# iamgroot42/A-LINK

Hardware: AMD Instinct MI355X
Metric: 112x112 face embeddings/sec (IR-ResNet-100 ArcFace, 512-d, L2-normalised) (higher is better)
Workload: dtype bf16

## Files before the change

a-link_amd/csrc/front_c64.hip:

```cpp
#include "conv_device.h"

namespace alink {
namespace {

typedef __attribute__((__vector_size__(4 * sizeof(int)))) int i32x4;

__device__ __forceinline__ void lds_done_then_barrier() {
    asm volatile("s_waitcnt lgkmcnt(0)\n\ts_barrier" ::: "memory");
}

template <int A>
struct IC { static constexpr int a = A; };

constexpr int NT = 256;
constexpr int W = 112, H = 112;
constexpr int P = 2;
constexpr int RING = 8;
constexpr int BR = 4;
constexpr int BPI = H / BR;
constexpr int PITCH = (W + 2) * 128;
constexpr int XBYTES = RING * PITCH;
constexpr int TBYTES = 11 * 64 * 4;
constexpr int IMPX = 32;
constexpr int IMROWB = W * IMPX;
constexpr int IMROWS = 8;
constexpr int TPWV = 7;
constexpr size_t lds_bytes() { return (size_t)XBYTES + TBYTES + IMROWS * IMROWB + 16; }

template <typename T, int LAYOUT, bool AMAX, bool STAMP>
__global__ __launch_bounds__(NT, 1) void front_c64_kernel(const ConvParams p, const StemParams s, T* __restrict__ xs) {
    typedef typename Vec8<T>::type vec8;
    auto prelu = [](float v, float slope) __attribute__((always_inline)) {
        const float w = v * slope;
        return AMAX ? __builtin_fmaxf(v, w) : (v > 0.f ? v : w);
    };
    extern __shared__ __attribute__((aligned(16))) char smem[];
    char* const imring = smem + XBYTES + TBYTES;

    const int tid = threadIdx.x, lane = tid & 63;
    const int wave = __builtin_amdgcn_readfirstlane(tid >> 6);
    const int ph = wave >> 1, ch = wave & 1;
    const int q = lane >> 4, lr = lane & 15;

    for (int i = tid; i < RING * 16; i += NT) {
        const int slot = i >> 4, side = (i >> 3) & 1, piece = i & 7;
        *(uint4*)(smem + slot * PITCH + (side ? (W + 1) * 128 : 0) + piece * 16) = uint4{0u, 0u, 0u, 0u};
    }
    for (int i = tid; i < IMROWS * IMROWB / 16; i += NT)
        *(uint4*)(imring + i * 16) = uint4{0u, 0u, 0u, 0u};
    float* const ebias = (float*)(smem + XBYTES);
    float* const ealpha = ebias + 9 * 64;
    for (int i = tid; i < 9 * 64; i += NT) ebias[i] = p.bias[i];
    float* const salpha = ealpha + 64;
    for (int i = tid; i < 64; i += NT) { ealpha[i] = p.alpha[i]; salpha[i] = s.alpha[i]; }

    const T* __restrict__ gw = (const T*)p.wgt;
    vec8 wr[2][9][2];
#pragma unroll
    for (int ct = 0; ct < 2; ++ct)
#pragma unroll
        for (int tap = 0; tap < 9; ++tap)
#pragma unroll
            for (int ks = 0; ks < 2; ++ks)
                wr[ct][tap][ks] = *(const vec8*)(gw + (size_t)(ch * 32 + 16 * ct + lr) * 576 + tap * 64 + ks * 32 + 8 * q);
    const int d = delta(lr);
    int loff[3][2];
#pragma unroll
    for (int kx = 0; kx < 3; ++kx)
#pragma unroll
        for (int ks = 0; ks < 2; ++ks)
            loff[kx][ks] = (d + kx) * 128 + ((((ks << 2) | q) ^ (((d + kx) >> 1) & 7)) << 4);

    vec8 swf[2][2];
#pragma unroll
    for (int t = 0; t < 2; ++t)
#pragma unroll
        for (int st = 0; st < 2; ++st) swf[t][st] = *(const vec8*)((const T*)s.wgt + (16 * (2 * ch + t) + lr) * 64 + st * 32 + 8 * q);
    float sbi[8];
#pragma unroll
    for (int i = 0; i < 8; ++i) sbi[i] = s.bias[16 * q + 8 * ch + i];
    const int rec_off = lr * IMPX + (q & 1) * 16;
    const int sw_off = (lr + 1) * 128 + (((2 * q + ch) ^ (((lr + 1) >> 1) & 7)) << 4);

    int goff[3], soff[3], prow[3];
    float ssub[3];
    {
        float sb0 = s.sub[0], sb1 = s.sub[1], sb2 = s.sub[2];
        asm volatile("" : "+s"(sb0), "+s"(sb1), "+s"(sb2));
#pragma unroll
        for (int jj = 0; jj < 3; ++jj) {
            const int i = tid + NT * jj;
            const bool valid = i < 672;
            const int r = i >= 336 ? 1 : 0, e = valid ? i - 336 * r : 0;
            int c, ix;
            if (LAYOUT == ALINK_LAYOUT_NCHW_F32) { c = e / W; ix = e - c * W; }
            else                                 { ix = e / 3; c = e - ix * 3; }
            const int cn = s.flip ? 2 - c : c;
            ssub[jj] = cn == 0 ? sb0 : (cn == 1 ? sb1 : sb2);
            goff[jj] = LAYOUT == ALINK_LAYOUT_NCHW_F32 ? c * H * W + ix : e;
            soff[jj] = valid ? (ix + 1) * IMPX + cn * 2 : -1;
            prow[jj] = r;
        }
    }
    constexpr int ROWP = LAYOUT == ALINK_LAYOUT_NCHW_F32 ? W : W * 3;
    char* const sink = imring + IMROWS * IMROWB;
    auto load_pair = [&](int n, int iy0, float (&raw)[3]) __attribute__((always_inline)) {
        const size_t base = (size_t)n * 3 * H * W;
#pragma unroll
        for (int jj = 0; jj < 3; ++jj) {
            int iy = iy0 + prow[jj];
            iy = iy < 0 ? 0 : (iy > H - 1 ? H - 1 : iy);
            const long long idx = (long long)base + iy * ROWP + goff[jj];
            if (LAYOUT == ALINK_LAYOUT_NHWC_U8) raw[jj] = (float)((const uint8_t*)s.in)[idx];
            else                                raw[jj] = ((const float*)s.in)[idx];
        }
    };
    auto store_pair = [&](int iy0, const float (&raw)[3]) __attribute__((always_inline)) {
        char* const rb0 = imring + ((iy0 + 8) & 7) * IMROWB;
        char* const rb1 = imring + ((iy0 + 9) & 7) * IMROWB;
#pragma unroll
        for (int jj = 0; jj < 3; ++jj) {
            const bool ok = (unsigned)(iy0 + prow[jj]) < (unsigned)H;
            const T v = (T)(ok ? (raw[jj] - ssub[jj]) * s.mul : 0.f);
            char* const dst = (prow[jj] ? rb1 : rb0) + soff[jj];
            *(T*)(soff[jj] >= 0 && soff[jj] < W * IMPX ? dst : sink) = v;
            *(T*)(soff[jj] >= 0 ? dst - IMPX + 6 : sink) = v;
            *(T*)(soff[jj] >= 2 * IMPX ? dst - 2 * IMPX + 12 : sink) = v;
        }
    };
    auto stem_rows = [&](int R0, int slot0, int n, int own_lo, int own_hi) __attribute__((always_inline)) {
        const int R = R0 + ph;
        int slot = slot0 + ph;
        if (slot >= RING) slot -= RING;
        const bool inimg = (unsigned)R < (unsigned)H;
        const char* const rbm = imring + ((R + 7) & 7) * IMROWB;
        const char* const rbz = imring + ((R + 8) & 7) * IMROWB;
        const char* const rbp = imring + ((R + 9) & 7) * IMROWB;
        const char* const wa = (q < 2 ? rbm : rbz) + rec_off;
        const char* const wb = rbp + rec_off;
        char* const ob = smem + slot * PITCH + sw_off;
        const bool to_xs = inimg && !(R & 1) && R >= own_lo && R < own_hi && !(lr & 1);
        T* const xrow = xs + ((size_t)(n * (H / 2) + (R >> 1)) * (W / 2) + (lr >> 1)) * 64 + 16 * q + 8 * ch;
        const int keep = inimg ? -1 : 0;
        const f32x4 sal0 = *(const f32x4*)(salpha + 16 * q + 8 * ch), sal1 = *(const f32x4*)(salpha + 16 * q + 8 * ch + 4);
        auto group = [&](auto X0, auto NX) __attribute__((always_inline)) {
            constexpr int x0 = decltype(X0)::a, nx = decltype(NX)::a;
            vec8 pa[nx], pb[nx];
#pragma unroll
            for (int i = 0; i < nx; ++i) {
                pa[i] = *(const vec8*)(wa + 16 * IMPX * (x0 + i));
                pb[i] = *(const vec8*)(wb + 16 * IMPX * (x0 + i));
            }
            f32x4 a0[nx], a1[nx];
#pragma unroll
            for (int i = 0; i < nx; ++i) {
                a0[i] = mfma16<T>(swf[0][0], pa[i], f32x4{sbi[0], sbi[1], sbi[2], sbi[3]});
                a1[i] = mfma16<T>(swf[1][0], pa[i], f32x4{sbi[4], sbi[5], sbi[6], sbi[7]});
            }
#pragma unroll
            for (int i = 0; i < nx; ++i) {
                a0[i] = mfma16<T>(swf[0][1], pb[i], a0[i]);
                a1[i] = mfma16<T>(swf[1][1], pb[i], a1[i]);
            }
#pragma unroll
            for (int i = 0; i < nx; ++i) {
                vec8 o8;
#pragma unroll
                for (int j = 0; j < 4; ++j) {
                    float v0 = a0[i][j], v1 = a1[i][j];
                    v0 = prelu(v0, sal0[j]);
                    v1 = prelu(v1, sal1[j]);
                    o8[j] = (T)v0;
                    o8[4 + j] = (T)v1;
                }
                i32x4 ob4 = __builtin_bit_cast(i32x4, o8);
#pragma unroll
                for (int j = 0; j < 4; ++j) ob4[j] &= keep;
                *(i32x4*)(ob + 2048 * (x0 + i)) = ob4;
                if (to_xs) *(i32x4*)(xrow + (size_t)(8 * (x0 + i)) * 64) = ob4;
            }
        };
        group(IC<0>{}, IC<4>{});
        group(IC<4>{}, IC<3>{});
    };

    auto compute = [&](f32x4 (&acc)[2][TPWV], int s0) __attribute__((always_inline)) {
#pragma unroll
        for (int ct = 0; ct < 2; ++ct)
#pragma unroll
            for (int u = 0; u < TPWV; ++u) acc[ct][u] = f32x4{0.f, 0.f, 0.f, 0.f};
        int sb[3];
#pragma unroll
        for (int ky = 0; ky < 3; ++ky) {
            int slot = s0 + ph + ky;
            if (slot >= RING) slot -= RING;
            sb[ky] = slot * PITCH;
        }
        vec8 pf[2][TPWV];
#pragma unroll
        for (int u = 0; u < TPWV; ++u) pf[0][u] = *(const vec8*)(smem + (sb[0] + loff[0][0]) + 2048 * u);
#pragma unroll
        for (int st = 0; st < 18; ++st) {
            if (st + 1 < 18) {
                const int tn = (st + 1) >> 1, ksn = (st + 1) & 1;
#pragma unroll
                for (int u = 0; u < TPWV; ++u)
                    pf[(st + 1) & 1][u] = *(const vec8*)(smem + (sb[tn / 3] + loff[tn % 3][ksn]) + 2048 * u);
            }
            const int tap = st >> 1, ks = st & 1;
#pragma unroll
            for (int ct = 0; ct < 2; ++ct)
#pragma unroll
                for (int u = 0; u < TPWV; ++u) acc[ct][u] = mfma16<T>(wr[ct][tap][ks], pf[st & 1][u], acc[ct][u]);
        }
    };
    auto epilogue = [&](const f32x4 (&acc)[2][TPWV], int y, long long img_row0) __attribute__((always_inline)) {
        const int rc = y == 0 ? 0 : (y == H - 1 ? 2 : 1);
        const size_t rowoff = (size_t)((img_row0 + y) * W) * 64 + ch * 32 + 8 * q;
        const f32x4 al0 = *(const f32x4*)(ealpha + ch * 32 + 8 * q), al1 = *(const f32x4*)(ealpha + ch * 32 + 8 * q + 4);
#pragma unroll
        for (int u = 0; u < TPWV; ++u) {
            const int x = 16 * u + d;
            const int cls = rc * 3 + (x == 0 ? 0 : (x == W - 1 ? 2 : 1));
            const f32x4 b0 = *(const f32x4*)(ebias + cls * 64 + ch * 32 + 8 * q);
            const f32x4 b1 = *(const f32x4*)(ebias + cls * 64 + ch * 32 + 8 * q + 4);
            float v[8];
#pragma unroll
            for (int j = 0; j < 4; ++j) { v[j] = acc[0][u][j] + b0[j]; v[4 + j] = acc[1][u][j] + b1[j]; }
#pragma unroll
            for (int i = 0; i < 8; ++i) v[i] = prelu(v[i], i < 4 ? al0[i & 3] : al1[i & 3]);
            vec8 o8;
#pragma unroll
            for (int i = 0; i < 8; ++i) o8[i] = (T)v[i];
            *(vec8*)((T*)p.out + rowoff + (size_t)x * 64) = o8;
        }
    };

    unsigned long long t_bar = 0, t_stem = 0, t_main = 0, t_pro = 0, t_a = 0, t_b = 0, t_c = 0, n_pass = 0;
    const unsigned long long t_start = STAMP ? __builtin_amdgcn_s_memtime() : 0;
    const long long nbands = (long long)p.N * BPI;
    const long long b0 = nbands * blockIdx.x / gridDim.x, b1 = nbands * (blockIdx.x + 1) / gridDim.x;
    for (long long band = b0; band < b1;) {
        const int n = (int)(band / BPI), j0 = (int)(band - (long long)n * BPI);
        int rb = BPI - j0;
        if (rb > b1 - band) rb = (int)(b1 - band);
        band += rb;
        const int y0 = j0 * BR, npass = rb * (BR / P), yend = y0 + rb * BR;
        const long long img_row0 = (long long)n * H;

        float raw[3];
        if (STAMP) t_a = __builtin_amdgcn_s_memtime();
        {
            float rawA[3], rawB[3], rawC[3];
            load_pair(n, y0 - 2, rawA);
            load_pair(n, y0, rawB);
            load_pair(n, y0 + 2, rawC);
            load_pair(n, y0 + 4, raw);
            lds_done_then_barrier();
            store_pair(y0 - 2, rawA);
            store_pair(y0, rawB);
            lds_done_then_barrier();
            store_pair(y0 + 2, rawC);
            stem_rows(y0 - 1, 0, n, y0, yend);
            lds_done_then_barrier();
            store_pair(y0 + 4, raw);
            load_pair(n, y0 + 6, raw);
            stem_rows(y0 + 1, 2, n, y0, yend);
        }
        int s0 = 0;
        f32x4 accA[2][TPWV], accB[2][TPWV];
        if (STAMP) t_pro += __builtin_amdgcn_s_memtime() - t_a;
        auto head = [&](int k) __attribute__((always_inline)) {
            if (STAMP) t_a = __builtin_amdgcn_s_memtime();
            lds_done_then_barrier();
            if (STAMP) { t_b = __builtin_amdgcn_s_memtime(); t_bar += t_b - t_a; }
            store_pair(y0 + 2 * k + 6, raw);
            load_pair(n, y0 + 2 * k + 8, raw);
            int sn = s0 + 4;
            if (sn >= RING) sn -= RING;
            stem_rows(y0 + 2 * k + 3, sn, n, y0, yend);
            if (STAMP) { t_c = __builtin_amdgcn_s_memtime(); t_stem += t_c - t_b; ++n_pass; }
            __builtin_amdgcn_sched_barrier(0);
        };
        auto advance = [&]() __attribute__((always_inline)) {
            if (STAMP) t_main += __builtin_amdgcn_s_memtime() - t_c;
            s0 += P;
            if (s0 >= RING) s0 -= RING;
        };
        head(0);
        compute(accA, s0);
        advance();
#pragma unroll 1
        for (int k = 1; k < npass; k += 2) {
            head(k);
            compute(accB, s0);
            epilogue(accA, y0 + (k - 1) * P + ph, img_row0);
            advance();
            if (k + 1 < npass) {
                head(k + 1);
                compute(accA, s0);
                epilogue(accB, y0 + k * P + ph, img_row0);
                    advance();
            } else {
                epilogue(accB, y0 + k * P + ph, img_row0);
            }
        }
    }
    if (STAMP && p.stamps && tid == 0) {
        unsigned long long* st = (unsigned long long*)p.stamps + (size_t)blockIdx.x * 8;
        st[0] = __builtin_amdgcn_s_memtime() - t_start; st[1] = t_bar; st[2] = t_stem; st[3] = t_main; st[4] = t_pro; st[5] = n_pass;
    }
}

bool g_fuse_stem = true;

}

extern "C" void alink_debug_set_fuse_stem(int on) { g_fuse_stem = on != 0; }

bool front_c64_applies(int dtype, int H_, int W_, int C0, int Cout) {
    return g_fuse_stem && (dtype == ALINK_DT_BF16 || dtype == ALINK_DT_F16) && H_ == H && W_ == W && C0 == 64 && Cout == 64;
}

template <typename T, int LAYOUT>
static hipError_t front_attr() {
    hipError_t e;
    if constexpr (LAYOUT == ALINK_LAYOUT_NHWC_U8) {
        e = hipFuncSetAttribute((const void*)front_c64_kernel<T, LAYOUT, true, true>, hipFuncAttributeMaxDynamicSharedMemorySize, (int)lds_bytes());
        if (e != hipSuccess) return e;
    }
    e = hipFuncSetAttribute((const void*)front_c64_kernel<T, LAYOUT, true, false>, hipFuncAttributeMaxDynamicSharedMemorySize, (int)lds_bytes());
    if (e != hipSuccess) return e;
    return hipFuncSetAttribute((const void*)front_c64_kernel<T, LAYOUT, false, false>, hipFuncAttributeMaxDynamicSharedMemorySize, (int)lds_bytes());
}
hipError_t front_c64_set_attributes() {
    hipError_t e;
    if ((e = front_attr<__bf16, ALINK_LAYOUT_NHWC_F32>()) != hipSuccess || (e = front_attr<__bf16, ALINK_LAYOUT_NCHW_F32>()) != hipSuccess ||
        (e = front_attr<__bf16, ALINK_LAYOUT_NHWC_U8>()) != hipSuccess)
        return e;
    if ((e = front_attr<_Float16, ALINK_LAYOUT_NHWC_F32>()) != hipSuccess || (e = front_attr<_Float16, ALINK_LAYOUT_NCHW_F32>()) != hipSuccess ||
        (e = front_attr<_Float16, ALINK_LAYOUT_NHWC_U8>()) != hipSuccess)
        return e;
    return hipSuccess;
}

template <typename T, int LAYOUT>
static void front_launch_l(const ConvParams& p, const StemParams& s, void* xs, bool amax, unsigned grid, hipStream_t st) {
    if (LAYOUT == ALINK_LAYOUT_NHWC_U8 && p.stamps && amax)
        hipLaunchKernelGGL((front_c64_kernel<T, ALINK_LAYOUT_NHWC_U8, true, true>), dim3(grid), dim3(NT), lds_bytes(), st, p, s, (T*)xs);
    else if (amax) hipLaunchKernelGGL((front_c64_kernel<T, LAYOUT, true, false>), dim3(grid), dim3(NT), lds_bytes(), st, p, s, (T*)xs);
    else           hipLaunchKernelGGL((front_c64_kernel<T, LAYOUT, false, false>), dim3(grid), dim3(NT), lds_bytes(), st, p, s, (T*)xs);
}
template <typename T>
static hipError_t front_launch(const ConvParams& p, const StemParams& s, void* xs, bool amax, unsigned grid, hipStream_t st) {
    switch (s.layout) {
        case ALINK_LAYOUT_NHWC_F32: front_launch_l<T, ALINK_LAYOUT_NHWC_F32>(p, s, xs, amax, grid, st); break;
        case ALINK_LAYOUT_NCHW_F32: front_launch_l<T, ALINK_LAYOUT_NCHW_F32>(p, s, xs, amax, grid, st); break;
        case ALINK_LAYOUT_NHWC_U8:  front_launch_l<T, ALINK_LAYOUT_NHWC_U8>(p, s, xs, amax, grid, st); break;
        default: return hipErrorInvalidValue;
    }
    return hipGetLastError();
}

hipError_t launch_front_c64(int dtype, const ConvParams& p, const StemParams& s, void* xs, bool slopes_le_1, hipStream_t st) {
    if (p.ksz != 3 || p.stride != 1 || p.pad != 1 || p.Cin != 64 || p.Cout != 64 || p.H != H || p.W != W) return hipErrorInvalidValue;
    if (s.H != H || s.W != W || s.C0 != 64 || s.N != p.N || p.N <= 0 || !xs) return hipErrorInvalidValue;
    if (p.splitk != 1 || p.dact || p.post_relu || p.in2 || p.resid || !p.alpha || !p.border_cls) return hipErrorInvalidValue;
    if ((long long)p.N * H * W * 64 >= (1ll << 31)) return hipErrorInvalidValue;
    const long long nbands = (long long)p.N * BPI;
    const unsigned grid = (unsigned)(nbands < 256 ? nbands : 256);
    if (dtype == ALINK_DT_BF16) return front_launch<__bf16>(p, s, xs, slopes_le_1, grid, st);
    if (dtype == ALINK_DT_F16)  return front_launch<_Float16>(p, s, xs, slopes_le_1, grid, st);
    return hipErrorInvalidValue;
}

}
```

Measured before the change: 45840.

## Warp-specialize fused stem/conv1 front kernel into producer and consumer waves

Doubles the block to 512 threads and splits it into four consumer waves that run the 3x3 conv MFMA loop and four producer waves that load the input image and compute stem rows into the LDS ring. The two roles step in lockstep through matching barrier counts, so stem work overlaps with conv compute instead of being serialized in each pass. The conv path drops the double-buffered accumulator scheme in favour of per-tile accumulators with explicit sched_group_barrier interleaving of LDS reads and MFMAs. The risks are the barrier matching between the two roles, register pressure at 512 threads with launch_bounds(…,1), and losing the epilogue/compute overlap.

```diff
diff --git a/a-link_amd/csrc/front_c64.hip b/a-link_amd/csrc/front_c64.hip
--- a/a-link_amd/csrc/front_c64.hip
+++ b/a-link_amd/csrc/front_c64.hip
@@ -12,7 +12,8 @@
 template <int A>
 struct IC { static constexpr int a = A; };
 
-constexpr int NT = 256;
+constexpr int NR = 256;
+constexpr int NT = 2 * NR;
 constexpr int W = 112, H = 112;
 constexpr int P = 2;
 constexpr int RING = 8;
@@ -24,35 +25,30 @@
 constexpr int IMPX = 32;
 constexpr int IMROWB = W * IMPX;
 constexpr int IMROWS = 8;
-constexpr int TPWV = 7;
 constexpr size_t lds_bytes() { return (size_t)XBYTES + TBYTES + IMROWS * IMROWB + 16; }
 
-template <typename T, int LAYOUT, bool AMAX, bool STAMP>
-__global__ __launch_bounds__(NT, 1) void front_c64_kernel(const ConvParams p, const StemParams s, T* __restrict__ xs) {
+template <bool AMAX>
+__device__ __forceinline__ float prelu(float v, float slope) {
+    const float w = v * slope;
+    return AMAX ? __builtin_fmaxf(v, w) : (v > 0.f ? v : w);
+}
+
+struct Run { int n, y0, npass, yend; };
+__device__ __forceinline__ Run next_run(long long& band, long long b1) {
+    const int n = (int)(band / BPI), j0 = (int)(band - (long long)n * BPI);
+    int rb = BPI - j0;
+    if (rb > b1 - band) rb = (int)(b1 - band);
+    band += rb;
+    return Run{n, j0 * BR, rb * (BR / P), j0 * BR + rb * BR};
+}
+
+template <typename T, bool AMAX, bool STAMP>
+__device__ __forceinline__ void front_conv1_wave(const ConvParams& p, char* smem, int wave, int lane, long long band, long long b1) {
     typedef typename Vec8<T>::type vec8;
-    auto prelu = [](float v, float slope) __attribute__((always_inline)) {
-        const float w = v * slope;
-        return AMAX ? __builtin_fmaxf(v, w) : (v > 0.f ? v : w);
-    };
-    extern __shared__ __attribute__((aligned(16))) char smem[];
-    char* const imring = smem + XBYTES + TBYTES;
-
-    const int tid = threadIdx.x, lane = tid & 63;
-    const int wave = __builtin_amdgcn_readfirstlane(tid >> 6);
     const int ph = wave >> 1, ch = wave & 1;
     const int q = lane >> 4, lr = lane & 15;
-
-    for (int i = tid; i < RING * 16; i += NT) {
-        const int slot = i >> 4, side = (i >> 3) & 1, piece = i & 7;
-        *(uint4*)(smem + slot * PITCH + (side ? (W + 1) * 128 : 0) + piece * 16) = uint4{0u, 0u, 0u, 0u};
-    }
-    for (int i = tid; i < IMROWS * IMROWB / 16; i += NT)
-        *(uint4*)(imring + i * 16) = uint4{0u, 0u, 0u, 0u};
-    float* const ebias = (float*)(smem + XBYTES);
-    float* const ealpha = ebias + 9 * 64;
-    for (int i = tid; i < 9 * 64; i += NT) ebias[i] = p.bias[i];
-    float* const salpha = ealpha + 64;
-    for (int i = tid; i < 64; i += NT) { ealpha[i] = p.alpha[i]; salpha[i] = s.alpha[i]; }
+    const float* const ebias = (const float*)(smem + XBYTES);
+    const float* const ealpha = ebias + 9 * 64;
 
     const T* __restrict__ gw = (const T*)p.wgt;
     vec8 wr[2][9][2];
@@ -64,12 +60,111 @@
             for (int ks = 0; ks < 2; ++ks)
                 wr[ct][tap][ks] = *(const vec8*)(gw + (size_t)(ch * 32 + 16 * ct + lr) * 576 + tap * 64 + ks * 32 + 8 * q);
     const int d = delta(lr);
+    const unsigned lane_o = d * 64 + ch * 32 + 8 * q;
     int loff[3][2];
 #pragma unroll
     for (int kx = 0; kx < 3; ++kx)
 #pragma unroll
         for (int ks = 0; ks < 2; ++ks)
             loff[kx][ks] = (d + kx) * 128 + ((((ks << 2) | q) ^ (((d + kx) >> 1) & 7)) << 4);
+
+    unsigned long long t_bar = 0, t_main = 0, t_pro = 0, t_a = 0, t_b = 0, n_pass = 0;
+    const unsigned long long t_start = STAMP ? __builtin_amdgcn_s_memtime() : 0;
+    while (band < b1) {
+        const Run r = next_run(band, b1);
+        const long long img_row0 = (long long)r.n * H;
+        if (STAMP) t_a = __builtin_amdgcn_s_memtime();
+        lds_done_then_barrier();
+        lds_done_then_barrier();
+        lds_done_then_barrier();
+        if (STAMP) t_pro += __builtin_amdgcn_s_memtime() - t_a;
+        int s0 = 0;
+#pragma unroll 1
+        for (int k = 0; k < r.npass; ++k) {
+            if (STAMP) t_a = __builtin_amdgcn_s_memtime();
+            lds_done_then_barrier();
+            if (STAMP) { t_b = __builtin_amdgcn_s_memtime(); t_bar += t_b - t_a; }
+            int sb[3];
+#pragma unroll
+            for (int ky = 0; ky < 3; ++ky) {
+                int slot = s0 + ph + ky;
+                if (slot >= RING) slot -= RING;
+                sb[ky] = slot * PITCH;
+            }
+            const int y = r.y0 + k * P + ph;
+            const int rc = y == 0 ? 0 : (y == H - 1 ? 2 : 1);
+            const unsigned rowoff = (unsigned)((img_row0 + y) * W) * 64u;
+            auto tiles = [&](auto X0, auto NX) __attribute__((always_inline)) {
+                constexpr int x0 = decltype(X0)::a, nx = decltype(NX)::a;
+                f32x4 acc[2][nx];
+#pragma unroll
+                for (int ct = 0; ct < 2; ++ct)
+#pragma unroll
+                    for (int u = 0; u < nx; ++u) acc[ct][u] = f32x4{0.f, 0.f, 0.f, 0.f};
+                vec8 pf[2][nx];
+#pragma unroll
+                for (int u = 0; u < nx; ++u) pf[0][u] = *(const vec8*)(smem + (sb[0] + loff[0][0]) + 2048 * (x0 + u));
+                __builtin_amdgcn_sched_barrier(0);
+#pragma unroll
+                for (int st = 0; st < 18; ++st) {
+                    if (st + 1 < 18) {
+                        const int tn = (st + 1) >> 1, ksn = (st + 1) & 1;
+#pragma unroll
+                        for (int u = 0; u < nx; ++u)
+                            pf[(st + 1) & 1][u] = *(const vec8*)(smem + (sb[tn / 3] + loff[tn % 3][ksn]) + 2048 * (x0 + u));
+                    }
+                    const int tap = st >> 1, ks = st & 1;
+#pragma unroll
+                    for (int ct = 0; ct < 2; ++ct)
+#pragma unroll
+                        for (int u = 0; u < nx; ++u) acc[ct][u] = mfma16<T>(wr[ct][tap][ks], pf[st & 1][u], acc[ct][u]);
+#pragma unroll
+                    for (int u = 0; u < nx; ++u) {
+                        if (st + 1 < 18) __builtin_amdgcn_sched_group_barrier(0x100, 1, 0);
+                        __builtin_amdgcn_sched_group_barrier(0x008, 2, 0);
+                    }
+                }
+                __builtin_amdgcn_sched_barrier(0);
+                const f32x4 al0 = *(const f32x4*)(ealpha + ch * 32 + 8 * q), al1 = *(const f32x4*)(ealpha + ch * 32 + 8 * q + 4);
+#pragma unroll
+                for (int u = 0; u < nx; ++u) {
+                    const int x = 16 * (x0 + u) + d;
+                    const int cls = rc * 3 + (x == 0 ? 0 : (x == W - 1 ? 2 : 1));
+                    const f32x4 bi0 = *(const f32x4*)(ebias + cls * 64 + ch * 32 + 8 * q);
+                    const f32x4 bi1 = *(const f32x4*)(ebias + cls * 64 + ch * 32 + 8 * q + 4);
+                    float v[8];
+#pragma unroll
+                    for (int j = 0; j < 4; ++j) { v[j] = acc[0][u][j] + bi0[j]; v[4 + j] = acc[1][u][j] + bi1[j]; }
+#pragma unroll
+                    for (int i = 0; i < 8; ++i) v[i] = prelu<AMAX>(v[i], i < 4 ? al0[i & 3] : al1[i & 3]);
+                    vec8 o8;
+#pragma unroll
+                    for (int i = 0; i < 8; ++i) o8[i] = (T)v[i];
+                    *(vec8*)((T*)p.out + (rowoff + 1024u * (x0 + u) + lane_o)) = o8;
+                }
+            };
+            tiles(IC<0>{}, IC<4>{});
+            tiles(IC<4>{}, IC<3>{});
+            if (STAMP) { t_main += __builtin_amdgcn_s_memtime() - t_b; ++n_pass; }
+            s0 += P;
+            if (s0 >= RING) s0 -= RING;
+        }
+    }
+    if (STAMP && p.stamps && wave == 0 && lane == 0) {
+        unsigned long long* st = (unsigned long long*)p.stamps + (size_t)blockIdx.x * 8;
+        st[0] = __builtin_amdgcn_s_memtime() - t_start; st[1] = t_bar; st[3] = t_main; st[4] = t_pro; st[5] = n_pass;
+    }
+}
+
+template <typename T, int LAYOUT, bool AMAX, bool STAMP>
+__device__ __forceinline__ void front_stem_wave(const ConvParams& p, const StemParams& s, T* __restrict__ xs, char* smem, int w, int rt, long long band,
+                                                long long b1) {
+    typedef typename Vec8<T>::type vec8;
+    char* const imring = smem + XBYTES + TBYTES;
+    const float* const salpha = (const float*)(smem + XBYTES) + 10 * 64;
+    const int lane = rt & 63;
+    const int ph = w >> 1, ch = w & 1;
+    const int q = lane >> 4, lr = lane & 15;
 
     vec8 swf[2][2];
 #pragma unroll
@@ -89,7 +184,7 @@
         asm volatile("" : "+s"(sb0), "+s"(sb1), "+s"(sb2));
 #pragma unroll
         for (int jj = 0; jj < 3; ++jj) {
-            const int i = tid + NT * jj;
+            const int i = rt + NR * jj;
             const bool valid = i < 672;
             const int r = i >= 336 ? 1 : 0, e = valid ? i - 336 * r : 0;
             int c, ix;
@@ -168,8 +263,8 @@
 #pragma unroll
                 for (int j = 0; j < 4; ++j) {
                     float v0 = a0[i][j], v1 = a1[i][j];
-                    v0 = prelu(v0, sal0[j]);
-                    v1 = prelu(v1, sal1[j]);
+                    v0 = prelu<AMAX>(v0, sal0[j]);
+                    v1 = prelu<AMAX>(v1, sal1[j]);
                     o8[j] = (T)v0;
                     o8[4 + j] = (T)v1;
                 }
@@ -184,72 +279,12 @@
         group(IC<4>{}, IC<3>{});
     };
 
-    auto compute = [&](f32x4 (&acc)[2][TPWV], int s0) __attribute__((always_inline)) {
-#pragma unroll
-        for (int ct = 0; ct < 2; ++ct)
-#pragma unroll
-            for (int u = 0; u < TPWV; ++u) acc[ct][u] = f32x4{0.f, 0.f, 0.f, 0.f};
-        int sb[3];
-#pragma unroll
-        for (int ky = 0; ky < 3; ++ky) {
-            int slot = s0 + ph + ky;
-            if (slot >= RING) slot -= RING;
-            sb[ky] = slot * PITCH;
-        }
-        vec8 pf[2][TPWV];
-#pragma unroll
-        for (int u = 0; u < TPWV; ++u) pf[0][u] = *(const vec8*)(smem + (sb[0] + loff[0][0]) + 2048 * u);
-#pragma unroll
-        for (int st = 0; st < 18; ++st) {
-            if (st + 1 < 18) {
-                const int tn = (st + 1) >> 1, ksn = (st + 1) & 1;
-#pragma unroll
-                for (int u = 0; u < TPWV; ++u)
-                    pf[(st + 1) & 1][u] = *(const vec8*)(smem + (sb[tn / 3] + loff[tn % 3][ksn]) + 2048 * u);
-            }
-            const int tap = st >> 1, ks = st & 1;
-#pragma unroll
-            for (int ct = 0; ct < 2; ++ct)
-#pragma unroll
-                for (int u = 0; u < TPWV; ++u) acc[ct][u] = mfma16<T>(wr[ct][tap][ks], pf[st & 1][u], acc[ct][u]);
-        }
-    };
-    auto epilogue = [&](const f32x4 (&acc)[2][TPWV], int y, long long img_row0) __attribute__((always_inline)) {
-        const int rc = y == 0 ? 0 : (y == H - 1 ? 2 : 1);
-        const size_t rowoff = (size_t)((img_row0 + y) * W) * 64 + ch * 32 + 8 * q;
-        const f32x4 al0 = *(const f32x4*)(ealpha + ch * 32 + 8 * q), al1 = *(const f32x4*)(ealpha + ch * 32 + 8 * q + 4);
-#pragma unroll
-        for (int u = 0; u < TPWV; ++u) {
-            const int x = 16 * u + d;
-            const int cls = rc * 3 + (x == 0 ? 0 : (x == W - 1 ? 2 : 1));
-            const f32x4 b0 = *(const f32x4*)(ebias + cls * 64 + ch * 32 + 8 * q);
-            const f32x4 b1 = *(const f32x4*)(ebias + cls * 64 + ch * 32 + 8 * q + 4);
-            float v[8];
-#pragma unroll
-            for (int j = 0; j < 4; ++j) { v[j] = acc[0][u][j] + b0[j]; v[4 + j] = acc[1][u][j] + b1[j]; }
-#pragma unroll
-            for (int i = 0; i < 8; ++i) v[i] = prelu(v[i], i < 4 ? al0[i & 3] : al1[i & 3]);
-            vec8 o8;
-#pragma unroll
-            for (int i = 0; i < 8; ++i) o8[i] = (T)v[i];
-            *(vec8*)((T*)p.out + rowoff + (size_t)x * 64) = o8;
-        }
-    };
-
-    unsigned long long t_bar = 0, t_stem = 0, t_main = 0, t_pro = 0, t_a = 0, t_b = 0, t_c = 0, n_pass = 0;
+    unsigned long long t_bar = 0, t_stem = 0, t_a = 0, t_b = 0;
     const unsigned long long t_start = STAMP ? __builtin_amdgcn_s_memtime() : 0;
-    const long long nbands = (long long)p.N * BPI;
-    const long long b0 = nbands * blockIdx.x / gridDim.x, b1 = nbands * (blockIdx.x + 1) / gridDim.x;
-    for (long long band = b0; band < b1;) {
-        const int n = (int)(band / BPI), j0 = (int)(band - (long long)n * BPI);
-        int rb = BPI - j0;
-        if (rb > b1 - band) rb = (int)(b1 - band);
-        band += rb;
-        const int y0 = j0 * BR, npass = rb * (BR / P), yend = y0 + rb * BR;
-        const long long img_row0 = (long long)n * H;
-
+    while (band < b1) {
+        const Run r = next_run(band, b1);
+        const int n = r.n, y0 = r.y0, yend = r.yend;
         float raw[3];
-        if (STAMP) t_a = __builtin_amdgcn_s_memtime();
         {
             float rawA[3], rawB[3], rawC[3];
             load_pair(n, y0 - 2, rawA);
@@ -267,49 +302,49 @@
             load_pair(n, y0 + 6, raw);
             stem_rows(y0 + 1, 2, n, y0, yend);
         }
-        int s0 = 0;
-        f32x4 accA[2][TPWV], accB[2][TPWV];
-        if (STAMP) t_pro += __builtin_amdgcn_s_memtime() - t_a;
-        auto head = [&](int k) __attribute__((always_inline)) {
+        int sn = 4;
+#pragma unroll 1
+        for (int k = 0; k < r.npass; ++k) {
             if (STAMP) t_a = __builtin_amdgcn_s_memtime();
             lds_done_then_barrier();
             if (STAMP) { t_b = __builtin_amdgcn_s_memtime(); t_bar += t_b - t_a; }
             store_pair(y0 + 2 * k + 6, raw);
             load_pair(n, y0 + 2 * k + 8, raw);
-            int sn = s0 + 4;
+            stem_rows(y0 + 2 * k + 3, sn, n, y0, yend);
+            if (STAMP) t_stem += __builtin_amdgcn_s_memtime() - t_b;
+            sn += P;
             if (sn >= RING) sn -= RING;
-            stem_rows(y0 + 2 * k + 3, sn, n, y0, yend);
-            if (STAMP) { t_c = __builtin_amdgcn_s_memtime(); t_stem += t_c - t_b; ++n_pass; }
-            __builtin_amdgcn_sched_barrier(0);
-        };
-        auto advance = [&]() __attribute__((always_inline)) {
-            if (STAMP) t_main += __builtin_amdgcn_s_memtime() - t_c;
-            s0 += P;
-            if (s0 >= RING) s0 -= RING;
-        };
-        head(0);
-        compute(accA, s0);
-        advance();
-#pragma unroll 1
-        for (int k = 1; k < npass; k += 2) {
-            head(k);
-            compute(accB, s0);
-            epilogue(accA, y0 + (k - 1) * P + ph, img_row0);
-            advance();
-            if (k + 1 < npass) {
-                head(k + 1);
-                compute(accA, s0);
-                epilogue(accB, y0 + k * P + ph, img_row0);
-                    advance();
-            } else {
-                epilogue(accB, y0 + k * P + ph, img_row0);
-            }
-        }
-    }
-    if (STAMP && p.stamps && tid == 0) {
+        }
+    }
+    if (STAMP && p.stamps && rt == 0) {
         unsigned long long* st = (unsigned long long*)p.stamps + (size_t)blockIdx.x * 8;
-        st[0] = __builtin_amdgcn_s_memtime() - t_start; st[1] = t_bar; st[2] = t_stem; st[3] = t_main; st[4] = t_pro; st[5] = n_pass;
-    }
+        st[2] = t_stem; st[6] = t_bar; st[7] = __builtin_amdgcn_s_memtime() - t_start;
+    }
+}
+
+template <typename T, int LAYOUT, bool AMAX, bool STAMP>
+__global__ __launch_bounds__(NT, 1) void front_c64_kernel(const ConvParams p, const StemParams s, T* __restrict__ xs) {
+    extern __shared__ __attribute__((aligned(16))) char smem[];
+    char* const imring = smem + XBYTES + TBYTES;
+    const int tid = threadIdx.x;
+    const int wave = __builtin_amdgcn_readfirstlane(tid >> 6);
+
+    for (int i = tid; i < RING * 16; i += NT) {
+        const int slot = i >> 4, side = (i >> 3) & 1, piece = i & 7;
+        *(uint4*)(smem + slot * PITCH + (side ? (W + 1) * 128 : 0) + piece * 16) = uint4{0u, 0u, 0u, 0u};
+    }
+    for (int i = tid; i < IMROWS * IMROWB / 16; i += NT)
+        *(uint4*)(imring + i * 16) = uint4{0u, 0u, 0u, 0u};
+    float* const ebias = (float*)(smem + XBYTES);
+    float* const ealpha = ebias + 9 * 64;
+    for (int i = tid; i < 9 * 64; i += NT) ebias[i] = p.bias[i];
+    float* const salpha = ealpha + 64;
+    for (int i = tid; i < 64; i += NT) { ealpha[i] = p.alpha[i]; salpha[i] = s.alpha[i]; }
+
+    const long long nbands = (long long)p.N * BPI;
+    const long long b0 = nbands * blockIdx.x / gridDim.x, b1 = nbands * (blockIdx.x + 1) / gridDim.x;
+    if (wave < 4) front_conv1_wave<T, AMAX, STAMP>(p, smem, wave, tid & 63, b0, b1);
+    else          front_stem_wave<T, LAYOUT, AMAX, STAMP>(p, s, xs, smem, wave - 4, tid - NR, b0, b1);
 }
 
 bool g_fuse_stem = true;
```

Result: no change. 46130, median of 6 (+0.6%).
